# watercore2001/BasicSR4RS

Hardware: AMD Instinct MI355X
Metric: HR-pixels/sec/node (x4 SR train step) + PSNR parity vs CPU ref (higher is better)
Workload: dtype bf16; 1 GPU; EDSR_Lx4 train step (32 RB, nf 256, res_scale 0.1), LR 64x64 -> HR 256x256; global_batch=32, per_gpu_batch=32, lr_tile=64, parallelism=dp1, model=EDSR, hip_graph=True, async_wgrad=False

## Files before the change

basicsr4rs_amd/csrc/conv3x3.hip:

```cpp
#include <cstdlib>
#include <utility>
#include <type_traits>
#include "sr_common.h"
#include "sr_internal.h"

namespace {

int g_variant = 0;
#define g_disable_big (g_variant == 1)

struct FwdArgs {
  const void* x;
  const void* w;
  const float* bias;
  const void* gate;
  const void* res;
  const float* aff_scale;
  const float* aff_shift;
  void* y;
  uint32_t x_bytes, w_bytes, g_bytes, r_bytes;
  int N, H, W, M;
  int Cin, ldx, xcoff, in_ps, cpt;
  int Cout, Cout_real, ldw, nkc;
  int ldy, ycoff, out_ps, out_nchw;
  int act;
  float slope, alpha;
  int ldg, gcoff;
  float gate_slope;
  int ldr, rcoff;
  float beta;
  const void* res2;
  uint32_t r2_bytes;
  int ldr2, r2coff, rcols;
  float beta2;
  int in_up;
  int tap0;
  int gate_mode;
  int gcol0, gcol1;
  void* aux;
  float* colsum;
  int tiles_n, tiles;
  FastDiv fd_cpt, fd_W, fd_H, fd_cps;
  FastDiv fd_r;
  unsigned long long* stamps;
  const float* row_scale;
  FastDiv fd_hw;
  const float* ln_g;
  const float* ln_b;
  void* ln_out;
  float* ln_mean;
  float* ln_rstd;
  int ln_C;
  float ln_eps;
  const void* dot;
  uint32_t d_bytes;
  int ldd, dcoff;
  int cs_band;
  int strip64;
};

SR_DEV float row_alpha(const FwdArgs& a, int m) {
  return a.row_scale ? a.alpha * a.row_scale[fdiv((uint32_t)m, a.fd_hw)] : a.alpha;
}

template <typename T>
SR_DEV void mfma_chunk(const u32x4& a, const u32x4& b, f32x4& acc);

template <>
SR_DEV void mfma_chunk<bf16_t>(const u32x4& a, const u32x4& b, f32x4& acc) {
  acc = __builtin_amdgcn_mfma_f32_16x16x32_bf16(__builtin_bit_cast(s16x8, a),
                                                __builtin_bit_cast(s16x8, b), acc, 0, 0, 0);
}
template <>
SR_DEV void mfma_chunk<float>(const u32x4& a, const u32x4& b, f32x4& acc) {
#pragma unroll
  for (int s = 0; s < 4; ++s)
    acc = __builtin_amdgcn_mfma_f32_16x16x4f32(__uint_as_float(a[s]), __uint_as_float(b[s]), acc,
                                               0, 0, 0);
}

SR_DEV uint32_t swz128(uint32_t r, uint32_t c) { return r * 128u + ((c ^ (r & 7u)) << 4); }

// ... 619 lines not shown
    __builtin_amdgcn_s_setprio(0);
  };

  if constexpr (FAST) k_eval();
  issue_a(0, 0);
  issue_b(0, 0);
  issue_b(0, 1);
  issue_a(0, 1);
  asm volatile("s_waitcnt vmcnt(4)" ::: "memory");
  pp_barrier();
  if (wr) pp_barrier();

  for (int t = 0; t < nk; ++t) {
    const int buf = t & 1;
    const bool more = t + 1 < nk;
    read_a(buf, 0);
    read_b(buf, 0);
    if (more) {
      if constexpr (FAST) k_advance();
      issue_a(t + 1, 0);
      asm volatile("s_waitcnt vmcnt(4)" ::: "memory");
    } else {
      asm volatile("s_waitcnt vmcnt(2)" ::: "memory");
    }
    pp_barrier();
    mma(0, 0);
    pp_barrier();
    read_b(buf, 1);
    if (more) {
      issue_b(t + 1, 0);
      asm volatile("s_waitcnt vmcnt(4)" ::: "memory");
    } else {
      asm volatile("s_waitcnt vmcnt(0)" ::: "memory");
    }
    pp_barrier();
    mma(0, 1);
    pp_barrier();
    read_a(buf, 1);
    if (more) issue_b(t + 1, 1);
    pp_barrier();
    mma(1, 1);
    pp_barrier();
    if (more) {
      issue_a(t + 1, 1);
      asm volatile("s_waitcnt vmcnt(4)" ::: "memory");
    }
    pp_barrier();
    mma(1, 0);
    pp_barrier();
  }
  if (!wr) pp_barrier();

  float* Cs = (float*)smem;
#pragma unroll
  for (int h = 0; h < 2; ++h) {
    __syncthreads();
#pragma unroll
    for (int g = 0; g < 2; ++g)
#pragma unroll
      for (int i = 0; i < 4; ++i)
#pragma unroll
        for (int j = 0; j < 2; ++j)
#pragma unroll
          for (int r = 0; r < 4; ++r)
            Cs[(wr * 64 + i * 16 + (lane >> 4) * 4 + r) * CSTR + g * 128 + wc * 32 + j * 16 + (lane & 15)] =
                acc[h][g][i][j][r];
    __syncthreads();
    epilogue_tile<bf16_t, 128, 256, 512>(a, Cs, CSTR, m0 + h * 128, n0, tid);
  }
}

constexpr int PPH_SLOT0 = 2 * 32768;
template <int R>
struct PphGeom {
  static constexpr int W = 256 / R;
  static constexpr int ROWB = (W + 2) * 128;
  static constexpr int NSLOT = R == 4 ? 11 : 5;
  static constexpr int PIECES = W / 64;
  static constexpr int ZERO = PPH_SLOT0 + NSLOT * ROWB;
  static constexpr int LDS = ZERO + 1024;
  static_assert(LDS <= 160 * 1024, "pph LDS");
};

template <int R, int P2 = 0, bool STRIP = false>
__global__ __launch_bounds__(512) void conv3x3_fwd_pph_kernel(FwdArgs a) {
  static_assert(!STRIP || (R == 4 && P2 == 2), "pph strips: the R 4 two-interval form");
  using G = PphGeom<R>;
  constexpr int W = G::W, RH = R + 2;
  constexpr int CSTR = 256 + 4;
  constexpr int SMEM = G::LDS > 128 * CSTR * 4 ? G::LDS : 128 * CSTR * 4;
  __shared__ __attribute__((aligned(16))) char smem[SMEM];

  const int tid = threadIdx.x, lane = tid & 63;
  const int w = __builtin_amdgcn_readfirstlane(tid >> 6);
  const int wr = w >> 2, wc = w & 3;
  const uint32_t tile = xcd_remap(blockIdx.x, gridDim.x);
  const int m0 = (int)(tile / a.tiles_n) * 256;
  const int n0 = (int)(tile % a.tiles_n) * 256;
  int img, y0, sx0 = 0;
  if constexpr (STRIP) {
    const int tm = m0 >> 8, tps = a.H >> 2, ns = a.W >> 6;
    img = tm / (tps * ns);
    const int rem = tm - img * tps * ns, j = rem / tps;
    y0 = (rem - j * tps) * 4;
    sx0 = j * 64;
  } else {
    const int HW = a.H * W;
    img = m0 / HW;
    y0 = (m0 - img * HW) / W;
  }
  const __amdgpu_buffer_rsrc_t xr = make_rsrc(a.x, a.x_bytes);
  const __amdgpu_buffer_rsrc_t wr_ = make_rsrc(a.w, a.w_bytes);

  const int c = (lane & 7) ^ (lane >> 3);
  const int ch_h = (lane & 7) ^ (((lane >> 3) + 1) & 7);
  uint32_t boff[4];
  bool bval[4];
#pragma unroll
  for (int k = 0; k < 4; ++k) {
    const int n = n0 + (k >> 1) * 128 + w * 16 + (k & 1) * 8 + (lane >> 3);
    bval[k] = n < a.Cout;
    boff[k] = (uint32_t)(n * a.ldw) * 2u + (uint32_t)c * 16u;
  }
  const int rps = a.in_ps > 0 ? a.in_ps : 1;
  const uint32_t hlane = (uint32_t)((sx0 + 8 * w + (lane >> 3)) * rps * a.ldx + a.xcoff) * 2u + (uint32_t)ch_h * 16u;
  const uint32_t rowb = (uint32_t)((STRIP ? a.W : W) * rps * rps * a.ldx) * 2u;
  const uint32_t pieceb = (uint32_t)(64 * rps * a.ldx) * 2u;
  auto chunk_off = [&](int cc) -> uint32_t {
    if (a.in_ps == 0) return (uint32_t)cc * 128u;
    const int c0 = cc * 64;
    const int sl = (int)fdiv((uint32_t)c0, a.fd_cps), cch = c0 - sl * a.fd_cps.d;
    const int si = sl / rps, sj = sl - si * rps;
    return (uint32_t)((si * W * rps + sj) * a.ldx + cch) * 2u;
  };

  if (tid < 64) *(u32x4*)(smem + G::ZERO + tid * 16) = u32x4{0u, 0u, 0u, 0u};
  if (!STRIP && tid < G::NSLOT * 16) {
    const int sl = tid >> 4, e = tid & 15;
    *(u32x4*)(smem + PPH_SLOT0 + sl * G::ROWB + (e < 8 ? 0 : (W + 1) * 128) + (e & 7) * 16) =
        u32x4{0u, 0u, 0u, 0u};
  }

  f32x4 acc[2][2][4][2];
#pragma unroll
  for (int h = 0; h < 2; ++h)
#pragma unroll
    for (int g = 0; g < 2; ++g)
#pragma unroll
      for (int i = 0; i < 4; ++i)
#pragma unroll
        for (int j = 0; j < 2; ++j) acc[h][g][i][j] = f32x4{0.f, 0.f, 0.f, 0.f};

  const int nchunk = a.Cin >> 6;
  const int nk = nchunk * 9;
  auto issue_dummy = [&]() { glds16(xr, smem + G::ZERO, SR_OOB); };
  auto issue_row = [&](int cc, int rr, int p) {
    const int y = y0 - 1 + rr;
    const int slot = (RH * cc + rr) % G::NSLOT;
    glds16(xr, smem + PPH_SLOT0 + slot * G::ROWB + 128 + p * 8192 + w * 1024,
           (unsigned)y < (unsigned)a.H
               ? (uint32_t)(img * a.H + y) * rowb + (uint32_t)p * pieceb + hlane + chunk_off(cc)
               : SR_OOB);
    if constexpr (STRIP) {
      if (w < 2) {
        const int q = (w == 0 ? 0 : W - 6) + (lane >> 3);
        const int sx = sx0 + q - 1;
        const int lcb = (lane & 7) ^ (q & 7);
        const bool v = (unsigned)y < (unsigned)a.H && (unsigned)sx < (unsigned)a.W;
        glds16(xr, smem + PPH_SLOT0 + slot * G::ROWB + (w == 0 ? 0 : (W - 6) * 128),
               v ? (uint32_t)(((img * a.H + y) * a.W + sx) * a.ldx + a.xcoff) * 2u + (uint32_t)lcb * 16u + chunk_off(cc)
                 : SR_OOB);
      } else {
        issue_dummy();
      }
    }
  };
  auto issue_halo_dummy = [&]() {
    issue_dummy();
    if constexpr (STRIP) issue_dummy();
  };
  auto issue_halo = [&](int cc, int j) {
    if constexpr (R == 4) {
      if (j < 6 && cc + 1 < nchunk) issue_row(cc + 1, j, 0); else issue_halo_dummy();
    } else {
      if (j < 2) issue_row(cc, 3, j);
      else if (j < 8 && cc + 1 < nchunk) issue_row(cc + 1, (j - 2) >> 1, j & 1);
      else issue_halo_dummy();
    }
  };
  auto issue_b = [&](int buf, int kc, int kt, int g) {
    char* dst = smem + buf * 32768 + g * 16384 + w * 2048;
    const uint32_t kofs = (uint32_t)(kt * a.Cin + kc * 64) * 2u;
#pragma unroll
    for (int j = 0; j < 2; ++j) {
      const int k = g * 2 + j;
      glds16(wr_, dst + j * 1024, bval[k] ? boff[k] + kofs : SR_OOB);
    }
  };
  auto issue_b_dummy = [&]() {
#pragma unroll
    for (int j = 0; j < 2; ++j) issue_dummy();
  };

  u32x4 fa[2][4], fb[2][2][2];
  auto qoff = [&](int tx, int kk) -> uint32_t {
    const uint32_t pxi = (uint32_t)((lane & 15) + tx);
    return pxi * 128u + ((((uint32_t)(kk * 4 + (lane >> 4))) ^ (pxi & 7u)) << 4);
  };
  const uint32_t q00 = qoff(0, 0), q01 = qoff(0, 1), q10 = qoff(1, 0), q11 = qoff(1, 1), q20 = qoff(2, 0),
                 q21 = qoff(2, 1);
  const int xoff = R == 4 ? 0 : wr * 64 * 128;
  auto read_a = [&](int slot, int tx) {
    const char* Rs = smem + PPH_SLOT0 + slot * G::ROWB + xoff;
#pragma unroll
    for (int kk = 0; kk < 2; ++kk) {
      const uint32_t qa = kk ? q01 : q00, qb = kk ? q11 : q10, qc = kk ? q21 : q20;
      const uint32_t qq = tx == 0 ? qa : (tx == 1 ? qb : qc);
#pragma unroll
      for (int i = 0; i < 4; ++i) fa[kk][i] = *(const u32x4*)(Rs + qq + i * 2048);
    }
  };
  auto read_b = [&](int buf, int g) {
    const char* Bs = smem + buf * 32768 + g * 16384;
#pragma unroll
    for (int kk = 0; kk < 2; ++kk)
#pragma unroll
      for (int j = 0; j < 2; ++j)
        fb[g][kk][j] = *(const u32x4*)(Bs + swz128(wc * 32 + j * 16 + (lane & 15), kk * 4 + (lane >> 4)));
  };
  auto mma = [&](int h, int g) {
    __builtin_amdgcn_s_setprio(1);
#pragma unroll
    for (int kk = 0; kk < 2; ++kk)
#pragma unroll
      for (int i = 0; i < 4; ++i)
#pragma unroll
        for (int j = 0; j < 2; ++j) mfma_chunk<bf16_t>(fa[kk][i], fb[g][kk][j], acc[h][g][i][j]);
    __builtin_amdgcn_s_setprio(0);
  };

#pragma unroll 1
  for (int rr = 0; rr < (R == 4 ? 6 : 3); ++rr)
#pragma unroll
    for (int p = 0; p < G::PIECES; ++p) issue_row(0, rr, p);
  issue_b(0, 0, 0, 0);
  issue_b(0, 0, 0, 1);
  if constexpr (P2 == 2) {
    if (nk > 1) { issue_b(1, 0, 1, 0); issue_b(1, 0, 1, 1); }
  }
  asm volatile("s_waitcnt vmcnt(0)" ::: "memory");
  pp_barrier();
  if (wr) pp_barrier();

  int cc = 0, tap = 0;
  int ncc = 0, ntap = 1;
  int n2cc = 0, n2tap = 2;
  if (n2tap == 9) { n2tap = 0; ++n2cc; }
#pragma unroll 1
  for (int t = 0; t < nk; ++t) {
    const int buf = t & 1;
    const bool more = t + 1 < nk;
    const int ty = tap / 3, tx = tap - ty * 3;
    int sa, sb;
    if constexpr (R == 4) {
      sa = (RH * cc + ty + wr) % G::NSLOT;
      sb = sa + 2;
    } else {
      sa = (RH * cc + ty) % G::NSLOT;
      sb = sa + 1;
    }
    if (sb >= G::NSLOT) sb -= G::NSLOT;
    if constexpr (P2 == 2) {
      read_a(sa, tx);
      read_b(buf, 0);
      read_b(buf, 1);
      asm volatile("s_waitcnt lgkmcnt(0)" ::: "memory");
      pp_barrier();
      mma(0, 0);
      mma(0, 1);
      pp_barrier();
      read_a(sb, tx);
      if (t + 2 < nk) { issue_b(buf, n2cc, n2tap, 0); issue_b(buf, n2cc, n2tap, 1); }
      else { issue_b_dummy(); issue_b_dummy(); }
      issue_halo(cc, tap);
      if constexpr (STRIP) {
        if (wr) asm volatile("s_waitcnt vmcnt(8)" ::: "memory");
      } else {
        if (wr) asm volatile("s_waitcnt vmcnt(6)" ::: "memory");
      }
      pp_barrier();
      mma(1, 1);
      mma(1, 0);
      if constexpr (STRIP) {
        if (!wr) asm volatile("s_waitcnt vmcnt(8)" ::: "memory");
      } else {
        if (!wr) asm volatile("s_waitcnt vmcnt(6)" ::: "memory");
      }
      pp_barrier();
      cc = ncc;
      tap = ntap;
      if (++ntap == 9) { ntap = 0; ++ncc; }
      if (++n2tap == 9) { n2tap = 0; ++n2cc; }
      continue;
    }
    if constexpr (P2 == 1) {
      read_a(sa, tx);
      read_b(buf, 0);
      read_b(buf, 1);
      if (more) { issue_b(buf ^ 1, ncc, ntap, 0); issue_b(buf ^ 1, ncc, ntap, 1); }
      else { issue_b_dummy(); issue_b_dummy(); }
      pp_barrier();
      mma(0, 0);
      mma(0, 1);
      pp_barrier();
      read_a(sb, tx);
      issue_halo(cc, tap);
      if (wr) asm volatile("s_waitcnt vmcnt(1)" ::: "memory");
      pp_barrier();
      mma(1, 1);
      mma(1, 0);
      if (!wr) asm volatile("s_waitcnt vmcnt(1)" ::: "memory");
      pp_barrier();
      cc = ncc;
      tap = ntap;
      if (++ntap == 9) { ntap = 0; ++ncc; }
      continue;
    }
    read_a(sa, tx);
    read_b(buf, 0);
    if (more) issue_b(buf ^ 1, ncc, ntap, 0); else issue_b_dummy();
    asm volatile("s_waitcnt vmcnt(3)" ::: "memory");
    pp_barrier();
    mma(0, 0);
    pp_barrier();
    read_b(buf, 1);
    if (more) issue_b(buf ^ 1, ncc, ntap, 1); else issue_b_dummy();
    pp_barrier();
    mma(0, 1);
    pp_barrier();
    read_a(sb, tx);
    issue_halo(cc, tap);
    pp_barrier();
    mma(1, 1);
    pp_barrier();
    asm volatile("s_waitcnt vmcnt(3)" ::: "memory");
    pp_barrier();
    mma(1, 0);
    pp_barrier();
    cc = ncc;
    tap = ntap;
    if (++ntap == 9) { ntap = 0; ++ncc; }
  }
  if (!wr) pp_barrier();
  asm volatile("s_waitcnt vmcnt(0)" ::: "memory");

  float* Cs = (float*)smem;
#pragma unroll
  for (int h = 0; h < 2; ++h) {
    __syncthreads();
#pragma unroll
    for (int g = 0; g < 2; ++g)
#pragma unroll
      for (int i = 0; i < 4; ++i)
#pragma unroll
        for (int j = 0; j < 2; ++j)
#pragma unroll
          for (int r = 0; r < 4; ++r)
            Cs[(wr * 64 + i * 16 + (lane >> 4) * 4 + r) * CSTR + g * 128 + wc * 32 + j * 16 + (lane & 15)] =
                acc[h][g][i][j][r];
    __syncthreads();
    epilogue_tile<bf16_t, 128, 256, 512>(a, Cs, CSTR, m0 + h * 128, n0, tid);
  }
}

template <int E>
__global__ __launch_bounds__(256, 2) void linear_wk_kernel(FwdArgs a) {
  constexpr int XI = 128 * 128, WI = 192 * 128, STAGE = XI + WI;
  constexpr int ACT = E & 3, GATE = (E >> 2) & 3;
  constexpr bool RES = (E & 16) != 0, AUX = (E & 64) != 0, RSC = (E & 128) != 0;
  static_assert(GATE != 3 && (E & ~(3 | 12 | 16 | 64 | 128)) == 0, "linear_wk: epilogue subset");
  __shared__ __attribute__((aligned(16))) char smem[2 * STAGE];
  const int tid = threadIdx.x, lane = tid & 63;
  const int w = __builtin_amdgcn_readfirstlane(tid >> 6);
  const int wr = w >> 1, wc = w & 1;
  const int nct = (a.Cout + 191) / 192;
  const int bt = (int)xcd_remap(blockIdx.x, gridDim.x);
  const int tt = bt / nct, ct = bt - tt * nct;
  const int m0 = tt * 128, n0 = ct * 192;
  const int K = a.Cin, nk = (K + 63) >> 6;
  const __amdgpu_buffer_rsrc_t xr = make_rsrc(a.x, a.x_bytes);
  const __amdgpu_buffer_rsrc_t wrs = make_rsrc(a.w, a.w_bytes);

  const int rl = lane >> 3, lc = (lane & 7) ^ rl;
  int wch[6];
#pragma unroll
  for (int q = 4; q < 10; ++q) {
    const int row = (w + 4 * q - 16) * 8 + rl;
    const int t = (row >> 4) & 1, r = row & 15;
    wch[q - 4] = n0 + (row >> 5) * 32 + 8 * (r >> 2) + 4 * t + (r & 3);
  }
  auto issue = [&](int ks, int stg) {
    char* st = smem + stg * STAGE;
    const int kc = ks * 8 + lc;
    const bool kv = kc * 8 < K;
#pragma unroll
    for (int q = 0; q < 4; ++q) {
      const int p = w + 4 * q, m = m0 + p * 8 + rl;
      glds16(xr, st + p * 1024, (kv && m < a.M) ? (uint32_t)((m * a.ldx + a.xcoff + kc * 8) * 2) : SR_OOB);
    }
#pragma unroll
    for (int q = 4; q < 10; ++q) {
      const int p = w + 4 * q - 16, ch = wch[q - 4];
      glds16(wrs, st + XI + p * 1024, (kv && ch < a.Cout) ? (uint32_t)((ch * a.ldw + kc * 8) * 2) : SR_OOB);
    }
  };

  const int c16 = lane & 15, g = lane >> 4;
  f32x4 acc[6][4];
#pragma unroll
  for (int i = 0; i < 6; ++i)
#pragma unroll
    for (int j = 0; j < 4; ++j) acc[i][j] = f32x4{0.f, 0.f, 0.f, 0.f};
  auto compute = [&](int stg) {
    const char* Xs = smem + stg * STAGE;
    const char* Ws = Xs + XI;
#pragma unroll
    for (int kk = 0; kk < 2; ++kk) {
      const int phys = ((kk * 4 + g) ^ (c16 & 7)) << 4;
      u32x4 fa[6], fb[4];
#pragma unroll
      for (int i = 0; i < 6; ++i) fa[i] = *(const u32x4*)(Ws + (wr * 96 + i * 16 + c16) * 128 + phys);
#pragma unroll
      for (int j = 0; j < 4; ++j) fb[j] = *(const u32x4*)(Xs + (wc * 64 + j * 16 + c16) * 128 + phys);
      __builtin_amdgcn_s_setprio(1);
#pragma unroll
      for (int i = 0; i < 6; ++i)
#pragma unroll
        for (int j = 0; j < 4; ++j)
          acc[i][j] = __builtin_amdgcn_mfma_f32_16x16x32_bf16(__builtin_bit_cast(s16x8, fa[i]),
                                                              __builtin_bit_cast(s16x8, fb[j]), acc[i][j], 0, 0, 0);
      __builtin_amdgcn_s_setprio(0);
    }
  };

  issue(0, 0);
  for (int ks = 0; ks < nk; ++ks) {
    asm volatile("s_waitcnt vmcnt(0)" ::: "memory");
    pp_barrier();
    if (ks + 1 < nk) issue(ks + 1, (ks + 1) & 1);
    compute(ks & 1);
  }

  const __amdgpu_buffer_rsrc_t rr = make_rsrc(a.res, a.r_bytes);
  const __amdgpu_buffer_rsrc_t gr = make_rsrc(a.gate, a.g_bytes);
// ... 2927 lines not shown
    const int cil = rem / taps, tap = rem - cil * taps;
    const int nn = n0 + nl, ci = c0 + cil;
    float v = 0.f;
    if (nn < it.Cout && ci < it.Cin) {
      const int co = row_of(nn);
      const int cs = it.col_map ? it.col_map[ci] : (ci < it.Cin_real ? ci : -1);
      if (co >= 0 && cs >= 0) v = it.w[((size_t)co * it.Cin_real + cs) * taps + tap];
    }
    tile[nl][tap][cil] = v;
  }
  if (it.bias_g && c0 == 0 && tid < PREP_T) {
    const int nn = n0 + tid;
    if (nn < it.Cout) {
      const int co = row_of(nn);
      it.bias_g[nn] = (co >= 0 && it.bias) ? it.bias[co] : 0.f;
    }
  }
  __syncthreads();
  T* wf = (T*)it.wf;
  T* wd = (T*)it.wd;
  if (Elt<T>::SIZE == 2 && it.Cin % 8 == 0 && it.Cout % 8 == 0) {
    constexpr int G8 = PREP_T / 8;
    for (int g = tid; g < PREP_T * taps * G8; g += 256) {
      const int a0 = g / (taps * G8), r = g - a0 * (taps * G8);
      const int tap = r / G8, e8 = (r - tap * G8) * 8;
      if (wf) {
        const int nn = n0 + a0, ci = c0 + e8;
        if (nn < it.Cout && ci < it.Cin) {
          u32x4 o;
#pragma unroll
          for (int j = 0; j < 4; ++j) o[j] = pack_bf16x2(tile[a0][tap][e8 + 2 * j], tile[a0][tap][e8 + 2 * j + 1]);
          *(u32x4*)(wf + (size_t)nn * taps * it.Cin + (size_t)tap * it.Cin + ci) = o;
        }
      }
      if (wd) {
        const int ci = c0 + a0, nn = n0 + e8;
        if (nn < it.Cout && ci < it.Cin) {
          u32x4 o;
#pragma unroll
          for (int j = 0; j < 4; ++j) o[j] = pack_bf16x2(tile[e8 + 2 * j][tap][a0], tile[e8 + 2 * j + 1][tap][a0]);
          *(u32x4*)(wd + (size_t)ci * taps * it.Cout + (size_t)(taps - 1 - tap) * it.Cout + nn) = o;
        }
      }
    }
    return;
  }
  for (int idx = tid; idx < PREP_T * per; idx += 256) {
    if (wf) {
      const int nl = idx / per, rem = idx - nl * per;
      const int tap = rem / PREP_T, cil = rem - tap * PREP_T;
      const int nn = n0 + nl, ci = c0 + cil;
      if (nn < it.Cout && ci < it.Cin) wf[(size_t)nn * taps * it.Cin + (size_t)tap * it.Cin + ci] = Elt<T>::from_f(tile[nl][tap][cil]);
    }
    if (wd) {
      const int cil = idx / per, rem = idx - cil * per;
      const int tap = rem / PREP_T, nl = rem - tap * PREP_T;
      const int nn = n0 + nl, ci = c0 + cil;
      if (nn < it.Cout && ci < it.Cin)
        wd[(size_t)ci * taps * it.Cout + (size_t)(taps - 1 - tap) * it.Cout + nn] = Elt<T>::from_f(tile[nl][tap][cil]);
    }
  }
}

template <typename T, int BM, int BN, int WM, int WN>
hipError_t launch_fwd(const FwdArgs& a0, hipStream_t s) {
  FwdArgs a = a0;
  const int tm = (a.M + BM - 1) / BM;
  a.tiles_n = (a.Cout + BN - 1) / BN;
  a.tiles = tm * a.tiles_n;
  hipLaunchKernelGGL((conv3x3_fwd_kernel<T, BM, BN, WM, WN>), dim3(a.tiles), dim3(256), 0, s, a);
  return hipGetLastError();
}

bool fwd_use_pph_strip(const FwdArgs& a) {
  return g_variant != 2 && g_variant != 24 && g_variant != 77 && a.W > 128 && a.W % 64 == 0 && a.H % 4 == 0 &&
         a.Cin % 64 == 0 && a.in_ps == 0 && a.in_up == 1 && a.tap0 == 0 && !a.colsum;
}
bool fwd_use_pph(const FwdArgs& a) {
  return g_variant != 2 && g_variant != 24 &&
         ((a.W == 64 && a.H % 4 == 0) || (a.W == 128 && a.H % 2 == 0)) && a.Cin % 64 == 0 &&
         (a.in_ps == 0 || (a.fd_cps.d % 64 == 0 && g_variant != 50)) && a.in_up == 1 && a.tap0 == 0;
}

hipError_t launch_fwd_big(const FwdArgs& a0, hipStream_t s) {
  FwdArgs a = a0;
  const int tm = (a.M + 255) / 256;
  a.tiles_n = (a.Cout + 255) / 256;
  a.tiles = tm * a.tiles_n;
  if (g_variant == 2)
    hipLaunchKernelGGL(conv3x3_fwd_big_kernel, dim3(a.tiles), dim3(512), 0, s, a);
  else if (fwd_use_pph_strip(a)) {
    a.strip64 = 1;
    hipLaunchKernelGGL((conv3x3_fwd_pph_kernel<4, 2, true>), dim3(a.tiles), dim3(512), 0, s, a);
  } else if (fwd_use_pph(a) && a.W == 128 && g_variant != 59)
    if (g_variant == 61) hipLaunchKernelGGL((conv3x3_fwd_pph_kernel<2, 1>), dim3(a.tiles), dim3(512), 0, s, a);
    else hipLaunchKernelGGL((conv3x3_fwd_pph_kernel<2, 2>), dim3(a.tiles), dim3(512), 0, s, a);
  else if (fwd_use_pph(a) && a.W == 128)
    hipLaunchKernelGGL((conv3x3_fwd_pph_kernel<2, 0>), dim3(a.tiles), dim3(512), 0, s, a);
  else if (g_variant != 59 && fwd_use_pph(a))
    if (g_variant == 61) hipLaunchKernelGGL((conv3x3_fwd_pph_kernel<4, 1>), dim3(a.tiles), dim3(512), 0, s, a);
    else hipLaunchKernelGGL((conv3x3_fwd_pph_kernel<4, 2>), dim3(a.tiles), dim3(512), 0, s, a);
  else if (fwd_use_pph(a))
    hipLaunchKernelGGL((conv3x3_fwd_pph_kernel<4, 0>), dim3(a.tiles), dim3(512), 0, s, a);
  else if ((a.Cin % 64 == 0 || a.tap0 == 4) && (a.in_ps == 0 || a.fd_cps.d % 64 == 0))
    hipLaunchKernelGGL(conv3x3_fwd_pp_kernel<true>, dim3(a.tiles), dim3(512), 0, s, a);
  else
    hipLaunchKernelGGL(conv3x3_fwd_pp_kernel<false>, dim3(a.tiles), dim3(512), 0, s, a);
  return hipGetLastError();
}

bool fwd_use_halo(const FwdArgs& a, bool bf) {
  const bool ps_ok = a.in_ps > 0 && a.fd_cps.d % 64 == 0 && a.W != 256 && g_variant != 68;
  if (!bf || a.in_up != 1 || (a.in_ps != 0 && !ps_ok) || a.tap0 != 0 || g_variant == 1) return false;
  if (a.W == 256)
    return a.Cout <= 16 && g_variant != 29;
  return !a.out_nchw && a.Cout < 256 && (a.W == 64 || a.W == 128) && a.H % (256 / a.W) == 0;
}

hipError_t launch_fwd_halo(const FwdArgs& a0, hipStream_t s) {
  FwdArgs a = a0;
  a.tiles_n = (a.Cout + 63) / 64;
  a.tiles = a.M / 256;
  const int ct = (a.Cout + 15) / 16;
  const dim3 grid(a.tiles, a.tiles_n);
  if (a.W == 256) hipLaunchKernelGGL((conv3x3_fwd_halo_kernel<1, true>), grid, dim3(256), 0, s, a);
  else if (ct == 1) hipLaunchKernelGGL(conv3x3_fwd_halo_kernel<1>, grid, dim3(256), 0, s, a);
  else if (ct == 2 && a.in_ps == 0)
    hipLaunchKernelGGL((conv3x3_fwd_halo_kernel<2, false, false, 3>), grid, dim3(256), 0, s, a);
  else if (ct == 2) hipLaunchKernelGGL(conv3x3_fwd_halo_kernel<2>, grid, dim3(256), 0, s, a);
  else if (!a.colsum && !a.out_nchw && a.out_ps == 0)
    hipLaunchKernelGGL((conv3x3_fwd_halo_kernel<4, false, true>), grid, dim3(256), 0, s, a);
  else hipLaunchKernelGGL(conv3x3_fwd_halo_kernel<4>, grid, dim3(256), 0, s, a);
  return hipGetLastError();
}

enum FwdKind { FK_HALO, FK_BIG, FK_256_16, FK_256_32, FK_128_64, FK_128_128, FK_LIN, FK_BAND, FK_TAIL, FK_BANDS };
int band_epi(const FwdArgs& a, int grid) {
  int gate = 0;
  if (a.gate) gate = a.gate_mode == 2 ? 3 : (a.gate_mode == 1 ? 2 : 1);
  const int e = a.act | (gate << 2) | (a.res ? 16 : 0) | (a.res2 ? 32 : 0) | (a.aux ? 64 : 0) |
                (a.colsum || a.dot ? 128 : 0) | (a.row_scale ? 256 : 0) | (a.dot ? 512 : 0);
  if (a.row_scale) {
    const int rows = (a.N * a.H + grid - 1) / grid;
    if ((rows + a.H - 1) / a.H + 1 > 64) return -1;
  }
  switch (e) {
    case 0: case 1: case 2: case 4: case 16: case 20: case 28: case 48: case 72: case 128: case 304: return e;
    case 656: return a.Cin == 64 && a.Cout == 64 ? e : -1;
    default: return -1;
  }
}
bool fwd_use_band(const FwdArgs& a, bool bf) {
  if (!(bf && a.tap0 == 0 && a.in_up == 1 && a.in_ps == 0 && !a.out_nchw && a.out_ps == 0 &&
        (a.W == 64 || a.W == 128) && (a.Cin == 32 || a.Cin == 64) && (a.Cout == 32 || a.Cout == 64) &&
        a.Cout_real == a.Cout && g_variant != 1 && g_variant != 34))
    return false;
  const int rows = a.N * a.H, gmax = g_variant == 35 ? 64 : 256;
  return band_epi(a, rows < gmax ? rows : gmax) >= 0;
}
bool fwd_use_band_strip(const FwdArgs& a, bool bf) {
  if (!(bf && a.tap0 == 0 && (a.in_up == 1 || a.in_up == 2) && a.in_ps == 0 && !a.out_nchw && a.out_ps == 0 &&
        a.W % 128 == 0 && (a.W > 128 || a.in_up == 2) && (a.Cin == 64 || (a.Cin <= 32 && a.Cin % 8 == 0)) &&
        (a.Cout == 64 || (a.Cin <= 32 && (a.Cout == 128 || a.Cout == 256))) && a.Cout_real == a.Cout &&
        !a.colsum && !a.dot && !a.row_scale && !a.res2 && !a.aux && g_variant != 1 && g_variant != 34 &&
        g_variant != 76))
    return false;
  const int e = band_epi(a, 256);
  if (a.Cout > 64) return e == 0;
  return a.Cin == 64 ? (e == 0 || e == 1 || e == 2 || e == 4) : (e == 0 || e == 4);
}
bool fwd_use_band_strip_sliced(const FwdArgs& a, bool bf) {
  if (!(a.Cout > 64 && a.Cout <= 256 && a.Cout % 64 == 0 && a.Cin <= 32) || fwd_use_band_strip(a, bf)) return false;
  FwdArgs b = a;
  b.Cout = b.Cout_real = 64;
  return fwd_use_band_strip(b, bf);
}
bool fwd_use_band_sliced(const FwdArgs& a, bool bf) {
  if (!(bf && a.tap0 == 0 && a.in_up == 1 && a.in_ps == 0 && !a.out_nchw && a.out_ps == 0 &&
        (a.W == 64 || a.W == 128) && (a.Cin == 32 || a.Cin == 64) && a.Cout > 64 && a.Cout < 256 &&
        a.Cout % 32 == 0 && a.Cout_real == a.Cout && !a.colsum && g_variant != 1 && g_variant != 34))
    return false;
  const int rows = a.N * a.H, gmax = g_variant == 35 ? 64 : 256;
  return band_epi(a, rows < gmax ? rows : gmax) >= 0;
// ... 569 lines not shown
    return sr_fail(SR_EINVAL, "linear_ln_fwd: null pointer");
  if (d->dtype != SR_BF16 || d->ksize != 1 || d->Cin % 8 || d->Cout % 8 || d->ldx != d->Cin || d->xcoff != 0 ||
      ln_C <= 0 || ln_C > d->Cin || d->ldw < d->Cin)
    return sr_fail(SR_EINVAL, "linear_ln_fwd: bf16 1x1 conv over dense rows (ldx == Cin) with ln_C <= Cin");
  FwdArgs a = fwd_shape(d);
  if (!fwd_use_lin(a, true) || a.Cin > 192)
    return sr_fail(SR_EINVAL, "linear_ln_fwd: shape not on the lin kernel (Cin <= 192, Cout <= 640)");
  a.aux = aux;
  const int e = lin_epi(a);
  if (e != 0 && e != 67) return sr_fail(SR_EINVAL, "linear_ln_fwd: epilogue must be plain or GELU + pre-activation aux");
  const size_t xb = (size_t)a.M * d->ldx * 2, wb = (size_t)d->Cout * d->ldw * 2;
  if (xb >= 0x80000000ull || wb >= 0x80000000ull) return sr_fail(SR_ETOOBIG, "linear_ln_fwd: tensor >= 2 GiB");
  a.x = x; a.w = w; a.bias = bias; a.y = y;
  a.x_bytes = (uint32_t)xb; a.w_bytes = (uint32_t)wb;
  a.ln_g = ln_gamma; a.ln_b = ln_beta; a.ln_out = ln_out; a.ln_mean = ln_mean; a.ln_rstd = ln_rstd;
  a.ln_C = ln_C; a.ln_eps = eps;
  a.tiles = (a.M + 127) / 128;
  hipStream_t s = (hipStream_t)stream;
#define SR_LNL(NP_)                                                                                       \
  case NP_:                                                                                               \
    if (e == 0) hipLaunchKernelGGL((conv3x3_lin_kernel<128, 3, NP_, 0, true>), dim3(a.tiles), dim3(256), 0, s, a); \
    else hipLaunchKernelGGL((conv3x3_lin_kernel<128, 3, NP_, 67, true>), dim3(a.tiles), dim3(256), 0, s, a); \
    break;
  switch ((a.Cout + 127) / 128) {
    SR_LNL(1) SR_LNL(2) SR_LNL(3) SR_LNL(4) SR_LNL(5)
    default: return sr_fail(SR_EINVAL, "linear_ln_fwd: Cout > 640");
  }
#undef SR_LNL
  return sr_check(hipGetLastError(), "linear_ln_fwd launch");
}

int sr_conv3x3_fwd_dot_ok(const sr_conv3x3_desc* d) {
  if (!d || d->N <= 0 || d->H <= 0 || d->W <= 0 || d->dtype != SR_BF16) return 0;
  FwdArgs a = fwd_shape(d);
  static const char one = 1;
  a.res = &one;
  a.dot = &one;
  a.colsum = (float*)&one;
  sr_conv3x3_desc dd = *d;
  dd.dot = &one;
  return fwd_kind(a, true) == FK_BAND && colsum_parts(&dd, a) > 0 ? 1 : 0;
}

int sr_conv3x3_fwd_colsum_parts(const sr_conv3x3_desc* d) {
  if (!d || d->N <= 0 || d->H <= 0 || d->W <= 0) return 0;
  return colsum_parts(d, fwd_shape(d));
}

const char* sr_conv3x3_fwd_kernel_name(const sr_conv3x3_desc* d) {
  const bool bf = d->dtype == SR_BF16;
  switch (fwd_kind(fwd_shape(d), bf)) {
    case FK_LIN: return lin_use_wk(fwd_shape(d)) ? "linear_wk_kernel" : "conv3x3_lin_kernel";
    case FK_HALO: return "conv3x3_fwd_halo_kernel";
    case FK_BAND: return "conv3x3_fwd_band_kernel";
    case FK_TAIL: return "conv3x3_fwd_tail_kernel";
    case FK_BANDS: return "conv3x3_fwd_band_kernel";
    case FK_BIG: {
      if (g_variant == 2) return "conv3x3_fwd_big_kernel";
      return fwd_use_pph(fwd_shape(d)) || fwd_use_pph_strip(fwd_shape(d)) ? "conv3x3_fwd_pph_kernel" : "conv3x3_fwd_pp_kernel";
    }
    case FK_256_16: return bf ? "conv3x3_fwd_kernel<bf16,256,16>" : "conv3x3_fwd_kernel<f32,256,16>";
    case FK_256_32: return bf ? "conv3x3_fwd_kernel<bf16,256,32>" : "conv3x3_fwd_kernel<f32,256,32>";
    case FK_128_64: return bf ? "conv3x3_fwd_kernel<bf16,128,64>" : "conv3x3_fwd_kernel<f32,128,64>";
    default: return bf ? "conv3x3_fwd_kernel<bf16,128,128>" : "conv3x3_fwd_kernel<f32,128,128>";
  }
}

int sr_conv3x3_fwd_launches(const sr_conv3x3_desc* d) {
  if (!d) return 0;
  const FwdArgs a = fwd_shape(d);
  return fwd_kind(a, d->dtype == SR_BF16) == FK_BANDS ? (a.Cout + 63) / 64 : 1;
}

const char* sr_conv3x3_wgrad_kernel_name(const sr_conv3x3_wgrad_desc* d) {
  if (wg_use_halo(d)) return "conv3x3_wgrad_ring_kernel";
  if (wg_use_lin(d)) return "linear_wgrad_kernel";
  if (wg_use_row3(d)) return "conv3x3_wgrad_row3_kernel";
  if (wg_use_pp(d)) return "conv3x3_wgrad_pp_kernel";
  if (wg_use_big(d)) return "conv3x3_wgrad_big_kernel";
  return d->dtype == SR_BF16 ? "conv3x3_wgrad_kernel<bf16>" : "conv3x3_wgrad_kernel<f32>";
}

int sr_conv3x3_set_variant(int variant) {
  static const int kValid[] = {0, 1, 2, 24, 28, 29, 33, 34, 35, 36, 37, 50, 55, 59, 61, 62, 63, 64, 67, 68, 76, 77, 78, 79};
  bool ok = false;
  for (int v : kValid) ok = ok || v == variant;
  if (!ok) return sr_fail(SR_EINVAL, "conv3x3_set_variant: not a parity cross-check variant");
  g_variant = variant;
  return SR_OK;
}

int sr_conv3x3_get_variant(void) { return g_variant; }

int sr_conv3x3_set_stamps(void* buf) {
  g_sr_stamps = (unsigned long long*)buf;
  return SR_OK;
}

size_t sr_conv3x3_wgrad_workspace(const sr_conv3x3_wgrad_desc* d) {
  int S, kp;
  wgrad_plan(d, &S, &kp);
  const int taps = d->ksize == 1 ? 1 : 9;
  return ((size_t)S * taps * d->Cout * d->Cin + (size_t)S * d->Cout) * sizeof(float) + 256;
}

}

namespace {
int wgrad_reduce_launch(const sr_conv3x3_wgrad_desc* d, int S, int taps, const float* ws, const float* wsb, float* dw,
                        float* db, const int* co_map, const int* ci_map, hipStream_t s) {
  const int acc1 = d->accumulate & 1;
  const int Cout_real = d->Cout_real > 0 ? d->Cout_real : d->Cout;
  const int Cin_real = d->Cin_real > 0 ? d->Cin_real : d->Cin;
  const int64_t total = (int64_t)Cout_real * Cin_real;
  const int64_t work = total > Cout_real ? total : Cout_real;
  const bool tr = wg_use_halo(d);
  const bool cig = !tr && ci_map && d->Cin % 4 == 0 && d->Cin <= 1024;
  if (!tr && ((Cin_real % 4 == 0 && !ci_map) || cig)) {
    const int64_t groups = tr ? (int64_t)taps * Cin_real * ((Cout_real + 3) / 4)
                              : (int64_t)taps * Cout_real * ((cig ? d->Cin : Cin_real) / 4);
    int P = 1;
    while (P * 8 < S && P < 32) P <<= 1;
    int gpw = 64;
    while (gpw > 16 && P * gpw / 64 > 16) gpw >>= 1;
    while (gpw > 16 && (groups + gpw - 1) / gpw < 256 && P * gpw / 64 >= 2) gpw >>= 1;
    const int nw = P * gpw / 64 > 0 ? P * gpw / 64 : 1;
    const int wblocks = (int)((groups + gpw - 1) / gpw);
    const int bblocks = db ? (Cout_real + 63) / 64 : 0;
    const dim3 grid((unsigned)(wblocks + bblocks)), blk((unsigned)(nw * 64));
#define SR_RG(G, T, ...)                                                                                        \
  hipLaunchKernelGGL((wgrad_reduce_g_kernel<G, T, ##__VA_ARGS__>), grid, blk, (size_t)nw * 64 * 16, s, (const float*)ws, (const float*)wsb, dw, db, \
                     S, d->Cout, d->Cin, Cout_real, Cin_real, d->out_ps, taps, co_map, ci_map, d->scale, wblocks,  \
                     acc1)
    if (tr) { if (gpw == 64) SR_RG(64, true); else if (gpw == 32) SR_RG(32, true); else SR_RG(16, true); }
    else if (cig) { if (gpw == 64) SR_RG(64, false, true); else if (gpw == 32) SR_RG(32, false, true); else SR_RG(16, false, true); }
    else { if (gpw == 64) SR_RG(64, false); else if (gpw == 32) SR_RG(32, false); else SR_RG(16, false); }
#undef SR_RG
  } else if (tr) {
    const int64_t work4 = (int64_t)taps * Cin_real * ((Cout_real + 3) / 4);
    const int wblocks = (int)((work4 + 63) / 64);
    const int bblocks = db ? (Cout_real + 63) / 64 : 0;
    hipLaunchKernelGGL(wgrad_reduce_tr_kernel, dim3((unsigned)(wblocks + bblocks)), dim3(1024), 0, s,
                       (const float*)ws, (const float*)wsb, dw, db, S, d->Cout, d->Cin, Cout_real, Cin_real, taps,
                       co_map, ci_map, d->scale, wblocks, acc1, d->out_ps);
  } else if (Cin_real % 4 == 0) {
    const int64_t work4 = (int64_t)taps * Cout_real * (Cin_real / 4);
    const int wblocks = (int)((work4 + 63) / 64);
    const int bblocks = db ? (Cout_real + 63) / 64 : 0;
    hipLaunchKernelGGL(wgrad_reduce4_kernel, dim3((unsigned)(wblocks + bblocks)), dim3(1024), 0, s, (const float*)ws,
                       (const float*)wsb, dw, db, S, d->Cout, d->Cin, Cout_real, Cin_real, d->out_ps, taps, co_map,
                       ci_map, d->scale, wblocks, acc1);
  } else if (Cin_real <= 8 && g_variant != 33) {
    hipLaunchKernelGGL(wgrad_reduce_narrow_kernel, dim3((unsigned)Cout_real), dim3(256), 0, s, (const float*)ws,
                       (const float*)wsb, dw, db, S, d->Cout, d->Cin, Cin_real, d->out_ps, taps, co_map, ci_map,
                       d->scale, acc1);
  } else {
    hipLaunchKernelGGL(wgrad_reduce_kernel, dim3((unsigned)((work + 255) / 256)), dim3(256), 0, s,
                       (const float*)ws, (const float*)wsb, dw, db, S, d->Cout, d->Cin, Cout_real,
                       Cin_real, d->out_ps, taps, co_map, ci_map, d->scale, acc1);
  }
  return sr_check(hipGetLastError(), "conv3x3_wgrad reduce launch");
}
}

extern "C" {

int sr_conv3x3_wgrad(const sr_conv3x3_wgrad_desc* d, const void* dy, const void* x, void* workspace,
// ... 147 lines not shown
```

basicsr4rs_amd/csrc/sr_core.hip:

```cpp
#include <stdio.h>
#include <stdlib.h>
#include <string.h>
#include <atomic>
#include <mutex>
#include "sr_internal.h"

static thread_local char g_err[512] = "";
unsigned long long* g_sr_stamps = nullptr;

int sr_fail(int code, const char* msg) {
  snprintf(g_err, sizeof(g_err), "%s", msg);
  return code;
}

int sr_check(hipError_t e, const char* what) {
  if (e == hipSuccess) return SR_OK;
  snprintf(g_err, sizeof(g_err), "%s: %s", what, hipGetErrorString(e));
  return SR_ELAUNCH;
}

static const char* const kKnobNames[K_COUNT] = {
    "SR_LWK", "SR_LWK_MINK", "SR_RING_WIDE", "SR_RING_PS", "SR_LWG", "SR_LWG_T", "SR_RING_SPLITS",
    "SR_DCN_CPP", "SR_DCN_DBG", "SR_DCN_R", "SR_DCN_FUSED", "SR_DCN_COORD_WIN",
    "SR_DCN_GX_FX", "SR_SWIN_ATTN_DBG", "SR_WG_ROW3"};
static std::atomic<int> g_knob[K_COUNT];
static std::once_flag g_knob_once;

static void knob_init() {
  for (int k = 0; k < K_COUNT; ++k) {
    const char* e = getenv(kKnobNames[k]);
    g_knob[k].store(e && *e ? atoi(e) : -1, std::memory_order_relaxed);
  }
}

int sr_knob(SrKnob k) {
  std::call_once(g_knob_once, knob_init);
  return g_knob[k].load(std::memory_order_relaxed);
}

static int knob_index(const char* name) {
  if (!name) return -1;
  for (int k = 0; k < K_COUNT; ++k)
    if (strcmp(kKnobNames[k], name) == 0) return k;
  return -1;
}

extern "C" int sr_set_knob(const char* name, int value, int* previous) {
  const int k = knob_index(name);
  if (k < 0) return sr_fail(SR_EINVAL, "set_knob: unknown knob name");
  std::call_once(g_knob_once, knob_init);
  const int old = g_knob[k].exchange(value < 0 ? -1 : value, std::memory_order_relaxed);
  if (previous) *previous = old;
  return SR_OK;
}

extern "C" int sr_get_knob(const char* name) {
  const int k = knob_index(name);
  return k < 0 ? -2 : sr_knob((SrKnob)k);
}

extern "C" const char* sr_version(void) { return "basicsr4rs_amd libsr_hip 0.2 (gfx950)"; }
extern "C" const char* sr_last_error(void) { return g_err; }
```

basicsr4rs_amd/csrc/sr_internal.h:

```cpp
#pragma once
#include <hip/hip_runtime.h>
#include "../../include/sr_hip.h"

int sr_fail(int code, const char* msg);
int sr_check(hipError_t e, const char* what);

enum SrKnob {
  K_LWK,
  K_LWK_MINK,
  K_RING_WIDE,
  K_RING_PS,
  K_LWG,
  K_LWG_T,
  K_RING_SPLITS,
  K_DCN_CPP,
  K_DCN_DBG,
  K_DCN_R,
  K_DCN_FUSED,
  K_DCN_COORD_WIN,
  K_DCN_GX_FX,
  K_SWIN_ATTN_DBG,
  K_WG_ROW3,
  K_COUNT
};
int sr_knob(SrKnob k);
extern unsigned long long* g_sr_stamps;
```

Before: 57.72 million HR-pixels/s.

## Add persistent pph conv3x3 forward kernel overlapping next-tile loads with epilogue

Adds a persistent variant of the R=4 two-interval pph forward conv kernel for 64-wide, 256-channel convs. The grid is capped at the CU count and each block loops over a contiguous range of tiles. While finishing one tile it prefetches the next tile's input rows and weights, and it runs a fused epilogue that stages through the LDS ring slots. The aim is to hide per-tile prologue and epilogue latency and the wave-quantization tail of the launch, at the cost of more complex slot bookkeeping. It also adds optional cycle-stamp instrumentation, a grid-size knob and an opt-out variant.

Result: faster. 60.03 million HR-pixels/s, median of 6 (+4.0%).

```diff
diff --git a/basicsr4rs_amd/csrc/conv3x3.hip b/basicsr4rs_amd/csrc/conv3x3.hip
--- a/basicsr4rs_amd/csrc/conv3x3.hip
+++ b/basicsr4rs_amd/csrc/conv3x3.hip
@@ -1,3 +1,4 @@
+#include <atomic>
 #include <cstdlib>
 #include <utility>
 #include <type_traits>
@@ -783,9 +784,18 @@
   static_assert(LDS <= 160 * 1024, "pph LDS");
 };
 
-template <int R, int P2 = 0, bool STRIP = false>
+template <int R, int P2 = 0, bool STRIP = false, bool PERS = false>
 __global__ __launch_bounds__(512) void conv3x3_fwd_pph_kernel(FwdArgs a) {
   static_assert(!STRIP || (R == 4 && P2 == 2), "pph strips: the R 4 two-interval form");
+  static_assert(!PERS || (R == 4 && P2 == 2 && !STRIP), "pph persistent: the R 4 two-interval form");
+#ifdef SR_BAND_STAMPS
+  const unsigned long long st_entry = __builtin_readcyclecounter();
+  unsigned long long* const st_p =
+      a.stamps && threadIdx.x == 0 && blockIdx.x < 4096 ? a.stamps + (size_t)blockIdx.x * 16 : nullptr;
+  auto stamp = [&](int ti, int k) {
+    if (st_p && ti < 3) st_p[2 + 4 * ti + k] = __builtin_readcyclecounter();
+  };
+#endif
   using G = PphGeom<R>;
   constexpr int W = G::W, RH = R + 2;
   constexpr int CSTR = 256 + 4;
@@ -940,6 +950,238 @@
     __builtin_amdgcn_s_setprio(0);
   };
 
+  if constexpr (PERS) {
+    constexpr int NS = G::NSLOT;
+    const int nb = (int)gridDim.x, run = (int)tile;
+    const int tq = a.tiles / nb, trem = a.tiles - tq * nb;
+    int tl = run * tq + (run < trem ? run : trem);
+    const int tend = tl + tq + (run < trem ? 1 : 0);
+    const int HW = a.H * W;
+    auto tile_pos = [&](int t_, int& im, int& yy) {
+      const int m = t_ * 256;
+      im = m / HW;
+      yy = (m - im * HW) / W;
+    };
+    int timg, ty0;
+    tile_pos(tl, timg, ty0);
+    auto issue_row_p = [&](int slot, int lc, int rr, int im, int yy0) {
+      const int y = yy0 - 1 + rr;
+      glds16(xr, smem + PPH_SLOT0 + slot * G::ROWB + 128 + w * 1024,
+             (unsigned)y < (unsigned)a.H ? (uint32_t)(im * a.H + y) * rowb + hlane + (uint32_t)lc * 128u : SR_OOB);
+    };
+    auto lds_sync = [&]() {
+      asm volatile("s_waitcnt lgkmcnt(0)" ::: "memory");
+      pp_barrier();
+    };
+    const bool useg = a.gate != nullptr;
+    const __amdgpu_buffer_rsrc_t orr = useg ? make_rsrc(a.gate, a.g_bytes) : make_rsrc(a.res, a.r_bytes);
+    const int e_cg = tid & 31, e_n = e_cg * 8, e_r0 = tid >> 5;
+    auto e_row = [](int q) { return (q >> 3) * 128 + (q & 1) * 64 + ((q >> 1) & 3) * 16; };
+    const bool e_oval = useg || (a.res && e_n < a.rcols);
+    const uint32_t e_ostep = (uint32_t)(useg ? a.ldg : a.ldr) * 2u;
+
+#pragma unroll 1
+    for (int rr = 0; rr < 6; ++rr) issue_row_p(rr, 0, rr, timg, ty0);
+    issue_b(0, 0, 0, 0);
+    issue_b(0, 0, 0, 1);
+    issue_b(1, 0, 1, 0);
+    issue_b(1, 0, 1, 1);
+    asm volatile("s_waitcnt vmcnt(0)" ::: "memory");
+    pp_barrier();
+    if (wr) pp_barrier();
+
+    int s0 = 0;
+    int par = 0;
+    int m0t = tl * 256;
+#ifdef SR_BAND_STAMPS
+    int sti = 0;
+    if (st_p) { st_p[0] = st_entry; st_p[1] = (unsigned long long)(tend - tl); }
+#endif
+#pragma unroll 1
+    for (; tl < tend; ++tl) {
+      const bool has_next = tl + 1 < tend;
+      int nimg = timg, ny0 = ty0;
+      if (has_next) tile_pos(tl + 1, nimg, ny0);
+#ifdef SR_BAND_STAMPS
+      stamp(sti, 0);
+#endif
+#pragma unroll
+      for (int h = 0; h < 2; ++h)
+#pragma unroll
+        for (int g = 0; g < 2; ++g)
+#pragma unroll
+          for (int i = 0; i < 4; ++i)
+#pragma unroll
+            for (int j = 0; j < 2; ++j) acc[h][g][i][j] = f32x4{0.f, 0.f, 0.f, 0.f};
+      int cc = 0, tap = 0;
+      int n2cc = 0, n2tap = 2;
+#pragma unroll 1
+      for (int t = 0; t < nk; ++t) {
+        const int buf = par;
+        par ^= 1;
+        const int ty = tap / 3, tx = tap - ty * 3;
+        int sa = s0 + ty + wr;
+        if (sa >= NS) sa -= NS;
+        int sb = sa + 2;
+        if (sb >= NS) sb -= NS;
+        read_a(sa, tx);
+        read_b(buf, 0);
+        read_b(buf, 1);
+        asm volatile("s_waitcnt lgkmcnt(0)" ::: "memory");
+        pp_barrier();
+        mma(0, 0);
+        mma(0, 1);
+        pp_barrier();
+        read_a(sb, tx);
+        if (t + 2 < nk || has_next) { issue_b(buf, n2cc, n2tap, 0); issue_b(buf, n2cc, n2tap, 1); }
+        else { issue_b_dummy(); issue_b_dummy(); }
+        {
+          const bool lastc = cc + 1 == nchunk;
+          if (tap < 6 && (!lastc || has_next)) {
+            int sl = s0 + 6 + tap;
+            if (sl >= NS) sl -= NS;
+            issue_row_p(sl, lastc ? 0 : cc + 1, tap, lastc ? nimg : timg, lastc ? ny0 : ty0);
+          } else {
+            issue_dummy();
+          }
+        }
+        if (wr) asm volatile("s_waitcnt vmcnt(6)" ::: "memory");
+        pp_barrier();
+        mma(1, 1);
+        mma(1, 0);
+        if (!wr) asm volatile("s_waitcnt vmcnt(6)" ::: "memory");
+        pp_barrier();
+        if (++tap == 9) {
+          tap = 0;
+          ++cc;
+          s0 += 6;
+          if (s0 >= NS) s0 -= NS;
+        }
+        if (++n2tap == 9) {
+          n2tap = 0;
+          if (++n2cc == nchunk) n2cc = 0;
+        }
+      }
+      u32x4 ova[8], ovb[8];
+      const uint32_t ob =
+          (uint32_t)(((size_t)(m0t + e_r0) * (useg ? a.ldg : a.ldr) + (useg ? a.gcoff : a.rcoff) + e_n) * 2);
+#pragma unroll
+      for (int q = 0; q < 8; ++q) ova[q] = buf_load16(orr, e_oval ? ob + (uint32_t)e_row(q) * e_ostep : SR_OOB);
+      f32x4 bias0 = f32x4{0.f, 0.f, 0.f, 0.f}, bias1 = bias0;
+      if (a.bias) {
+        bias0 = *(const f32x4*)(a.bias + e_n);
+        bias1 = *(const f32x4*)(a.bias + e_n + 4);
+      }
+      if (!wr) pp_barrier();
+#ifdef SR_BAND_STAMPS
+      stamp(sti, 1);
+#endif
+#pragma unroll
+      for (int p = 0; p < 8; ++p) {
+        const int h = p >> 2, i = p & 3;
+        if (p) lds_sync();
+        {
+          int sl = s0 + 6 + wr * 2 + (lane >> 5);
+          if (sl >= NS) sl -= NS;
+          float* Cw = (float*)(smem + PPH_SLOT0 + sl * G::ROWB) + (((lane >> 4) & 1) * 4) * CSTR + wc * 32 + (lane & 15);
+#pragma unroll
+          for (int g = 0; g < 2; ++g)
+#pragma unroll
+            for (int j = 0; j < 2; ++j)
+#pragma unroll
+              for (int r = 0; r < 4; ++r) Cw[r * CSTR + g * 128 + j * 16] = acc[h][g][i][j][r];
+        }
+        lds_sync();
+        if (p == 0) {
+#ifdef SR_BAND_STAMPS
+          const unsigned long long tw0 = __builtin_readcyclecounter();
+#endif
+          asm volatile("s_waitcnt vmcnt(0)" ::: "memory");
+#ifdef SR_BAND_STAMPS
+          if (st_p && sti < 3) st_p[14] += __builtin_readcyclecounter() - tw0;
+#endif
+        }
+#pragma unroll
+        for (int k2 = 0; k2 < 2; ++k2) {
+          const int q = p * 2 + k2;
+          int sl = s0 + 6 + k2 * 2 + (tid >> 8);
+          if (sl >= NS) sl -= NS;
+          const float* Cr = (const float*)(smem + PPH_SLOT0 + sl * G::ROWB) + (e_r0 & 7) * CSTR + e_cg * 8;
+          {
+            const int m = m0t + e_r0 + e_row(q);
+            float v[8];
+            const f32x4 c0 = *(const f32x4*)Cr;
+            const f32x4 c1 = *(const f32x4*)(Cr + 4);
+#pragma unroll
+            for (int j = 0; j < 4; ++j) { v[j] = c0[j]; v[4 + j] = c1[j]; }
+            if (a.bias) {
+#pragma unroll
+              for (int j = 0; j < 4; ++j) { v[j] += bias0[j]; v[4 + j] += bias1[j]; }
+            }
+            act_apply_n(v, a.act, a.slope);
+            u32x4 ovq = q < 8 ? ova[q & 7] : ovb[q & 7];
+            asm volatile("" : "+v"(ovq));
+            float o8[8];
+#pragma unroll
+            for (int j = 0; j < 4; ++j) {
+              const uint32_t oq = ovq[j];
+              o8[2 * j] = bf16_to_f32(oq & 0xffff);
+              o8[2 * j + 1] = bf16_to_f32(oq >> 16);
+            }
+            if (useg) {
+              if (a.gate_mode == 1) {
+#pragma unroll
+                for (int j = 0; j < 8; ++j) v[j] *= o8[j];
+              } else {
+#pragma unroll
+                for (int j = 0; j < 8; ++j) v[j] *= (o8[j] > 0.f ? 1.f : a.gate_slope);
+              }
+            }
+            {
+              const float al = a.alpha;
+#pragma unroll
+              for (int j = 0; j < 8; ++j) v[j] *= al;
+            }
+            if (!useg && a.res && e_n < a.rcols) {
+#pragma unroll
+              for (int j = 0; j < 8; ++j) v[j] = a.beta * o8[j] + v[j];
+            }
+            u32x4 o;
+#pragma unroll
+            for (int j = 0; j < 4; ++j) o[j] = pack_bf16x2(v[2 * j], v[2 * j + 1]);
+            *(u32x4*)((bf16_t*)a.y + ((size_t)m * a.ldy + a.ycoff + e_n)) = o;
+          }
+        }
+        if (p == 1) {
+#pragma unroll
+          for (int q = 0; q < 8; ++q) ovb[q] = buf_load16(orr, e_oval ? ob + (uint32_t)e_row(8 + q) * e_ostep : SR_OOB);
+        }
+#ifdef SR_BAND_STAMPS
+        if (p == 3) stamp(sti, 2);
+        if (p == 7) stamp(sti, 3);
+#endif
+      }
+#ifdef SR_BAND_STAMPS
+      ++sti;
+#endif
+      if (has_next) {
+        lds_sync();
+        if (tid < 64) {
+          int sl = s0 + 6 + (tid >> 4);
+          if (sl >= NS) sl -= NS;
+          const int e = tid & 15;
+          *(u32x4*)(smem + PPH_SLOT0 + sl * G::ROWB + (e < 8 ? 0 : (W + 1) * 128) + (e & 7) * 16) = u32x4{0u, 0u, 0u, 0u};
+        }
+        m0t += 256;
+        timg = nimg;
+        ty0 = ny0;
+        pp_barrier();
+        if (wr) pp_barrier();
+      }
+    }
+    return;
+  }
+
 #pragma unroll 1
   for (int rr = 0; rr < (R == 4 ? 6 : 3); ++rr)
 #pragma unroll
@@ -951,6 +1193,10 @@
   }
   asm volatile("s_waitcnt vmcnt(0)" ::: "memory");
   pp_barrier();
+#ifdef SR_BAND_STAMPS
+  if (st_p) { st_p[0] = st_entry; st_p[1] = 1; }
+  stamp(0, 0);
+#endif
   if (wr) pp_barrier();
 
   int cc = 0, tap = 0;
@@ -1054,6 +1300,9 @@
   }
   if (!wr) pp_barrier();
   asm volatile("s_waitcnt vmcnt(0)" ::: "memory");
+#ifdef SR_BAND_STAMPS
+  stamp(0, 1);
+#endif
 
   float* Cs = (float*)smem;
 #pragma unroll
@@ -1071,6 +1320,9 @@
                 acc[h][g][i][j][r];
     __syncthreads();
     epilogue_tile<bf16_t, 128, 256, 512>(a, Cs, CSTR, m0 + h * 128, n0, tid);
+#ifdef SR_BAND_STAMPS
+    stamp(0, 2 + h);
+#endif
   }
 }
 
@@ -4164,11 +4416,31 @@
          (a.in_ps == 0 || (a.fd_cps.d % 64 == 0 && g_variant != 50)) && a.in_up == 1 && a.tap0 == 0;
 }
 
+int device_cus() {
+  static std::atomic<int> cus[64];
+  int dev = 0;
+  if (hipGetDevice(&dev) != hipSuccess || dev < 0 || dev >= 64) dev = 0;
+  int n = cus[dev].load(std::memory_order_relaxed);
+  if (n <= 0) {
+    if (hipDeviceGetAttribute(&n, hipDeviceAttributeMultiprocessorCount, dev) != hipSuccess || n <= 0) n = 256;
+    cus[dev].store(n, std::memory_order_relaxed);
+  }
+  return n;
+}
+int pph_pers_grid(const FwdArgs& a) {
+  if (g_variant == 80 || a.W != 64 || a.Cout != 256 || a.tiles_n != 1 || a.in_ps != 0 || a.out_ps != 0 || a.colsum || a.out_nchw ||
+      a.aux || a.res2 || a.row_scale || a.dot || (a.gate && a.res) || (a.gate && a.gate_mode == 2) || a.M % 256)
+    return 0;
+  const int G = sr_knob(K_PPH_GRID) > 0 ? sr_knob(K_PPH_GRID) : device_cus();
+  return a.tiles > G ? G : 0;
+}
+
 hipError_t launch_fwd_big(const FwdArgs& a0, hipStream_t s) {
   FwdArgs a = a0;
   const int tm = (a.M + 255) / 256;
   a.tiles_n = (a.Cout + 255) / 256;
   a.tiles = tm * a.tiles_n;
+  a.stamps = g_sr_stamps;
   if (g_variant == 2)
     hipLaunchKernelGGL(conv3x3_fwd_big_kernel, dim3(a.tiles), dim3(512), 0, s, a);
   else if (fwd_use_pph_strip(a)) {
@@ -4181,6 +4453,8 @@
     hipLaunchKernelGGL((conv3x3_fwd_pph_kernel<2, 0>), dim3(a.tiles), dim3(512), 0, s, a);
   else if (g_variant != 59 && fwd_use_pph(a))
     if (g_variant == 61) hipLaunchKernelGGL((conv3x3_fwd_pph_kernel<4, 1>), dim3(a.tiles), dim3(512), 0, s, a);
+    else if (const int gp = pph_pers_grid(a))
+      hipLaunchKernelGGL((conv3x3_fwd_pph_kernel<4, 2, false, true>), dim3(gp), dim3(512), 0, s, a);
     else hipLaunchKernelGGL((conv3x3_fwd_pph_kernel<4, 2>), dim3(a.tiles), dim3(512), 0, s, a);
   else if (fwd_use_pph(a))
     hipLaunchKernelGGL((conv3x3_fwd_pph_kernel<4, 0>), dim3(a.tiles), dim3(512), 0, s, a);
@@ -4916,7 +5190,7 @@
 }
 
 int sr_conv3x3_set_variant(int variant) {
-  static const int kValid[] = {0, 1, 2, 24, 28, 29, 33, 34, 35, 36, 37, 50, 55, 59, 61, 62, 63, 64, 67, 68, 76, 77, 78, 79};
+  static const int kValid[] = {0, 1, 2, 24, 28, 29, 33, 34, 35, 36, 37, 50, 55, 59, 61, 62, 63, 64, 67, 68, 76, 77, 78, 79, 80};
   bool ok = false;
   for (int v : kValid) ok = ok || v == variant;
   if (!ok) return sr_fail(SR_EINVAL, "conv3x3_set_variant: not a parity cross-check variant");
diff --git a/basicsr4rs_amd/csrc/sr_core.hip b/basicsr4rs_amd/csrc/sr_core.hip
--- a/basicsr4rs_amd/csrc/sr_core.hip
+++ b/basicsr4rs_amd/csrc/sr_core.hip
@@ -22,7 +22,7 @@
 static const char* const kKnobNames[K_COUNT] = {
     "SR_LWK", "SR_LWK_MINK", "SR_RING_WIDE", "SR_RING_PS", "SR_LWG", "SR_LWG_T", "SR_RING_SPLITS",
     "SR_DCN_CPP", "SR_DCN_DBG", "SR_DCN_R", "SR_DCN_FUSED", "SR_DCN_COORD_WIN",
-    "SR_DCN_GX_FX", "SR_SWIN_ATTN_DBG", "SR_WG_ROW3"};
+    "SR_DCN_GX_FX", "SR_SWIN_ATTN_DBG", "SR_WG_ROW3", "SR_PPH_GRID"};
 static std::atomic<int> g_knob[K_COUNT];
 static std::once_flag g_knob_once;
 
diff --git a/basicsr4rs_amd/csrc/sr_internal.h b/basicsr4rs_amd/csrc/sr_internal.h
--- a/basicsr4rs_amd/csrc/sr_internal.h
+++ b/basicsr4rs_amd/csrc/sr_internal.h
@@ -21,6 +21,7 @@
   K_DCN_GX_FX,
   K_SWIN_ATTN_DBG,
   K_WG_ROW3,
+  K_PPH_GRID,
   K_COUNT
 };
 int sr_knob(SrKnob k);
```
